# djene-mengistu/UAPS

Measured on AMD Instinct MI355X. Metric: training images/sec (labeled+unlabeled) NEU-Seg 256x256 K=3, higher is better.
Workload: dtype f32

## Files before the change

### include/uaps_hip.h

```cpp
#ifndef UAPS_HIP_H
#define UAPS_HIP_H

#include <stddef.h>
#include <stdint.h>

#ifdef __cplusplus
extern "C" {
#endif

typedef void* uaps_stream_t;

#define UAPS_MAX_HEADS 8
#define UAPS_MAX_CLASSES 8

#define UAPS_OK 0
#define UAPS_EINVAL (-1)
#define UAPS_ERANGE (-2)
#define UAPS_EWORKSPACE (-3)
#define UAPS_ENOFORM (-4)

int uaps_abi_version(void);
const char* uaps_error_string(int code);


// ... 412 lines not shown
    float focal_alpha, focal_gamma;
    int focal_mean;
    float beta;
    float tversky_alpha, tversky_beta, eps;
} uaps_binloss_params;
#define UAPS_BIN_S_TERM 0
#define UAPS_BIN_S_LOSS 7
#define UAPS_BIN_S_BAD 8
#define UAPS_BIN_S_N 9
#define UAPS_BIN_S_P 10
#define UAPS_BIN_S_G 11
#define UAPS_BIN_S_I 12
#define UAPS_BIN_S_GP 13
#define UAPS_BIN_S_GI 14
#define UAPS_BIN_S_KBCE 15
#define UAPS_BIN_S_KFOCAL 16
#define UAPS_BIN_S_NSCALARS 24
int uaps_binloss_workspace_bytes(int B, int H, int W, size_t* out_host);
int uaps_binloss_fwd(const float* z, const void* target, const uaps_binloss_params* prm, int B, int H, int W, float* scalars,
                     void* workspace, size_t workspace_bytes, uaps_stream_t stream);
int uaps_binloss_bwd(const float* z, const void* target, const uaps_binloss_params* prm, const float* scalars, const float* grad,
                     int B, int H, int W, float* dz, uaps_stream_t stream);
int uaps_sigmoid_mse_fwd(const float* a, const float* b, long n, float* out, uaps_stream_t stream);
int uaps_sigmoid_mse_bwd(const float* a, const float* b, const float* g_map, long n, float* da, uaps_stream_t stream);
int uaps_sigmoid_kl_fwd(const float* a, const float* b, long n, float* out_mean, void* workspace, size_t workspace_bytes,
                        uaps_stream_t stream);
int uaps_sigmoid_kl_bwd(const float* a, const float* b, const float* grad, long n, float* da, uaps_stream_t stream);
int uaps_bin_confusion(const float* z, const int64_t* labels, int B, int H, int W, double threshold, int64_t* counts,
                       uaps_stream_t stream);

int uaps_add_relu(const float* a, const float* b, float* out, long n, uaps_stream_t stream);
int uaps_relu_bwd(const float* dout, const float* out, float* dx, long n, uaps_stream_t stream);
int uaps_bn_act_bwd_prepare(const float* dout, const float* y, const float* gamma, const float* beta, const float* save_mean,
                            const float* save_invstd, float slope, int B, int C, int H, int W, int groups, float* coef,
                            float* dgamma, float* dbeta, float* dconv_bias, float* dy_bound, void* workspace, size_t workspace_bytes,
                            uaps_stream_t stream);
int uaps_bn_act_bwd_finalize(const void* partials, int parts_per_image, const float* maxes, const float* gamma, const float* beta,
                             const float* save_mean, const float* save_invstd, int B, int C, int H, int W, int groups, float* coef,
                             float* dgamma, float* dbeta, float* dconv_bias, float* dy_bound, uaps_stream_t stream);
int uaps_bn_act_bwd_apply(const float* dout, const float* y, const float* coef, float slope, int B, int C, int H, int W, int groups,
                          float* dy, uaps_stream_t stream);
int uaps_head_bwd_fused(const float* dlogits, const float* y, const void* xf, float slope, int groups, const float* wb,
                        const float* dy_bound, float dy_mul, const float* x_bound, float x_mul, const float* save_mean,
                        const float* save_invstd, const float* gamma, const float* beta, int want_bias, int B, int Cin, int Cout,
                        int H, int W, int ks, int cfg, float* g, void* partials, float* maxes, void* workspace,
                        size_t workspace_bytes, uaps_stream_t stream);

int uaps_mid_bwd_fused(const float* dact, const float* y2, const float* coef, float slope2, int groups2, const float* y1,
                       const void* xf, float slope, int groups, const float* wb, const float* dy_bound, float dy_mul,
                       const float* x_bound, float x_mul, const float* save_mean, const float* save_invstd, const float* gamma,
                       const float* beta, int want_bias, int B, int Cin, int Cout, int H, int W, int ks, int cfg, float* g,
                       void* partials, float* maxes, void* workspace, size_t workspace_bytes, uaps_stream_t stream);

int uaps_relu_bwd_sum(const float* const* dout_host, int k, const float* out, float* dx, long n, uaps_stream_t stream);

int uaps_cat2(const float* a, const float* b, float* out, long n, uaps_stream_t stream);

int uaps_augment_batch(const uint8_t* images_hwc, const uint8_t* masks, const int* params_i, const float* params_f,
                       const float* noise, uint64_t seed, int B, int Hs, int Ws, int Ho, int Wo, const float* mean3_host,
                       const float* std3_host, float* out, int64_t* out_mask, uaps_stream_t stream);

#define UAPS_AUG_END 0
#define UAPS_AUG_BC 1
#define UAPS_AUG_NOISE 2
#define UAPS_AUG_BLUR 3
#define UAPS_AUG_BRIGHT 4
#define UAPS_AUG_CONTRAST 5
#define UAPS_AUG_SATURATE 6
#define UAPS_AUG_HUE 7
#define UAPS_AUG_PIXDROP 8
#define UAPS_AUG_GRID 9
#define UAPS_AUG_MAX_OPS 8
typedef struct uaps_view_row {
    int32_t hflip, vflip, rot_k, grid_on;
    int32_t op[UAPS_AUG_MAX_OPS];
    float a[UAPS_AUG_MAX_OPS], b[UAPS_AUG_MAX_OPS];
} uaps_view_row;
typedef struct uaps_augment_views_call {
    uint32_t struct_size;
    int32_t V, B, Hs, Ws, Cs, Ho, Wo;
    const uint8_t* images;
    const uint8_t* masks;
    const uaps_view_row* rows_host;
    const uaps_view_row* rows;
    const float* grid_ys;
    const float* grid_xs;
    const float* noise;
    const float* drop_u;
    uint64_t seed;
    float mean[3], std[3];
    float* out;
    int64_t* out_mask;
    void* workspace;
    size_t workspace_bytes;
    uaps_stream_t stream;
} uaps_augment_views_call;
int uaps_augment_views_workspace_bytes(int V, int B, int Ho, int Wo, size_t* bytes);
int uaps_augment_views(const uaps_augment_views_call* call);

int uaps_adam_step(float* const* params_host, const float* const* grads_host, float* const* exp_avg_host,
                   float* const* exp_avg_sq_host, const long* numel_host, int n, double lr, double beta1, double beta2,
                   double eps, double weight_decay, long step, uaps_stream_t stream);

int uaps_seg_confusion(const float* logits, const int64_t* labels, int B, int C, int H, int W,
                       int64_t* counts, uaps_stream_t stream);

// ... 261 lines not shown
```

### uaps_amd/_lib.py

```python
from __future__ import annotations

import ctypes as C
import os
import subprocess
import threading

from . import config

_HERE = os.path.dirname(os.path.abspath(__file__))
LIB_PATH = config.text("UAPS_HIP_LIB") or os.path.join(_HERE, "lib", "libuaps_hip.so")
CSRC = os.path.join(_HERE, "csrc")

_lock = threading.Lock()
_tls = threading.local()
_lib = None

c_float_p = C.POINTER(C.c_float)
c_void_p = C.c_void_p

_PTR = C.c_void_p
SIGNATURES = {
    "uaps_abi_version": (C.c_int, []),
    "uaps_error_string": (C.c_char_p, [C.c_int]),
    "uaps_loss_workspace_bytes": (C.c_int, [C.c_int] * 5 + [C.POINTER(C.c_size_t)]),
# ... 47 lines not shown
    "uaps_conv_fwd_bn": (C.c_int, [_PTR, _PTR, C.c_float, C.c_int] + [_PTR] * 4 + [C.c_int] * 7 + [_PTR]),
    "uaps_conv_bwd_weight_partial_bn": (C.c_int, [_PTR, _PTR, _PTR, C.c_float, C.c_int] + [C.c_int] * 8 + [_PTR, C.c_size_t, _PTR]),
    "uaps_conv_fwd_variant": (C.c_int, [C.c_int] * 7 + [C.c_char_p, C.c_size_t]),
    "uaps_conv_wrw_variant": (C.c_int, [C.c_int] * 7 + [C.c_char_p, C.c_size_t]),
    "uaps_conv_bwd_weight": (C.c_int, [_PTR] * 4 + [C.c_int] * 7 + [_PTR, C.c_size_t, _PTR]),
    "uaps_set_step_state": (C.c_int, [_PTR]),
    "uaps_next_call_hints": (C.c_int, [_PTR]),
    "uaps_conv_ex": (C.c_int, [_PTR]),
    "uaps_conv_ex_variant": (C.c_int, [_PTR, C.c_char_p, C.c_size_t]),
    "uaps_account": (C.c_int, [C.c_int]),
    "uaps_accounted_bytes": (C.c_double, []),
    "uaps_next_launch_events": (C.c_int, [_PTR, _PTR]),
    "uaps_zero_bounds": (C.c_int, [_PTR, C.c_long, _PTR]),
    "uaps_bn_param_bounds": (C.c_int, [_PTR, _PTR, _PTR, C.c_int, _PTR, _PTR]),
    "uaps_get_step_state": (C.c_void_p, []),
    "uaps_convs_pack_floats": (C.c_int, [C.c_int] * 3 + [C.POINTER(C.c_size_t), C.POINTER(C.c_size_t)]),
    "uaps_convs_pack_weights": (C.c_int, [_PTR] + [C.c_int] * 3 + [_PTR, _PTR, _PTR]),
    "uaps_convs_out_size": (C.c_int, [C.c_int] * 5 + [C.POINTER(C.c_int), C.POINTER(C.c_int)]),
    "uaps_convs_fwd": (C.c_int, [_PTR] * 3 + [C.c_int] * 8 + [_PTR]),
    "uaps_convs_bwd_data": (C.c_int, [_PTR] * 3 + [C.c_int] * 8 + [_PTR]),
    "uaps_convs_wrw_workspace_bytes": (C.c_int, [C.c_int] * 8 + [C.POINTER(C.c_size_t)]),
    "uaps_convs_bwd_weight": (C.c_int, [_PTR] * 3 + [C.c_int] * 8 + [_PTR, C.c_size_t, _PTR]),
    "uaps_maxpool3x3s2_fwd": (C.c_int, [_PTR, _PTR, _PTR, C.c_long, C.c_int, C.c_int, _PTR]),
    "uaps_maxpool3x3s2_bwd": (C.c_int, [_PTR, _PTR, _PTR, C.c_long, C.c_int, C.c_int, _PTR]),
    "uaps_space_to_depth2": (C.c_int, [_PTR, _PTR, C.c_int, C.c_int, C.c_int, C.c_int, C.c_int, _PTR]),
    "uaps_subsample2_fwd": (C.c_int, [_PTR, _PTR, C.c_long, C.c_int, C.c_int, _PTR]),
    "uaps_subsample2_bwd": (C.c_int, [_PTR, _PTR, C.c_long, C.c_int, C.c_int, _PTR]),
    "uaps_sum_tensors": (C.c_int, [_PTR, C.c_int, _PTR, C.c_long, _PTR]),
    "uaps_pair_workspace_bytes": (C.c_int, [C.POINTER(C.c_size_t)]),
    "uaps_feat_dropout_stats": (C.c_int, [_PTR] + [C.c_int] * 4 + [_PTR, C.c_size_t, _PTR]),
    "uaps_fanout_perturbed": (C.c_int, [_PTR] * 7 + [C.c_int, C.c_int, C.c_uint64, C.c_float, C.c_float] + [C.c_int] * 4 + [_PTR]),
    "uaps_augment_batch": (C.c_int, [_PTR] * 5 + [C.c_uint64] + [C.c_int] * 5 + [C.POINTER(C.c_float), C.POINTER(C.c_float), _PTR, _PTR, _PTR]),
    "uaps_augment_views_workspace_bytes": (C.c_int, [C.c_int] * 4 + [C.POINTER(C.c_size_t)]),
    "uaps_augment_views": (C.c_int, [_PTR]),
    "uaps_softmax_klmap_bwd": (C.c_int, [_PTR] * 3 + [C.c_int] * 4 + [_PTR] * 3),
    "uaps_softmax_pair_fwd": (C.c_int, [_PTR, _PTR] + [C.c_int] * 5 + [_PTR, _PTR, _PTR, _PTR, C.c_size_t, _PTR]),
    "uaps_softmax_mse_bwd": (C.c_int, [_PTR] * 3 + [C.c_int] * 4 + [_PTR, _PTR]),
    "uaps_softmax_kl_bwd": (C.c_int, [_PTR] * 3 + [C.c_int] * 4 + [_PTR, _PTR]),
    "uaps_entropy_map": (C.c_int, [_PTR] + [C.c_int] * 4 + [_PTR, _PTR, _PTR, C.c_size_t, _PTR]),
    "uaps_fanin_perturbed": (C.c_int, [_PTR] * 4 + [C.c_int, C.c_int, C.c_uint64, C.c_float, C.c_float] + [C.c_int] * 4 + [_PTR, _PTR]),
    "uaps_maxpool2x2_fwd": (C.c_int, [_PTR] + [C.c_int] * 4 + [_PTR, _PTR, _PTR]),
    "uaps_adam_step": (C.c_int, [_PTR] * 5 + [C.c_int] + [C.c_double] * 5 + [C.c_long, _PTR]),
    "uaps_add_relu": (C.c_int, [_PTR, _PTR, _PTR, C.c_long, _PTR]),
    "uaps_relu_bwd": (C.c_int, [_PTR, _PTR, _PTR, C.c_long, _PTR]),
    "uaps_relu_bwd_sum": (C.c_int, [_PTR, C.c_int, _PTR, _PTR, C.c_long, _PTR]),
    "uaps_cat2": (C.c_int, [_PTR, _PTR, _PTR, C.c_long, _PTR]),
    "uaps_bn_act_bwd_prepare": (C.c_int, [_PTR] * 6 + [C.c_float] + [C.c_int] * 5 + [_PTR] * 6 + [C.c_size_t, _PTR]),
    "uaps_bn_act_bwd_apply": (C.c_int, [_PTR] * 3 + [C.c_float] + [C.c_int] * 5 + [_PTR, _PTR]),
    "uaps_bn_act_bwd_finalize": (C.c_int, [_PTR, C.c_int] + [_PTR] * 5 + [C.c_int] * 5 + [_PTR] * 6),
    "uaps_head_bwd_fused": (C.c_int, [_PTR] * 3 + [C.c_float, C.c_int, _PTR, _PTR, C.c_float, _PTR, C.c_float] + [_PTR] * 4 + [C.c_int] * 8 +
                            [_PTR] * 4 + [C.c_size_t, _PTR]),
    "uaps_mid_bwd_fused": (C.c_int, [_PTR] * 3 + [C.c_float, C.c_int, _PTR, _PTR, C.c_float, C.c_int, _PTR, _PTR, C.c_float, _PTR, C.c_float] +
                           [_PTR] * 4 + [C.c_int] * 8 + [_PTR] * 4 + [C.c_size_t, _PTR]),
    "uaps_seg_confusion": (C.c_int, [_PTR, _PTR] + [C.c_int] * 4 + [_PTR, _PTR]),
    "uaps_ema_update": (C.c_int, [_PTR] * 3 + [C.c_int, C.c_float, C.c_float, _PTR]),
    "uaps_teacher_noise": (C.c_int, [_PTR] + [C.c_int] * 5 + [C.c_uint64, C.c_uint64, _PTR, _PTR]),
    "uaps_teacher_noise_apply": (C.c_int, [_PTR, _PTR] + [C.c_int] * 5 + [_PTR, _PTR]),
    "uaps_mc_consistency_workspace_bytes": (C.c_int, [C.POINTER(C.c_size_t)]),
    "uaps_mc_consistency_fwd": (C.c_int, [_PTR] * 3 + [C.c_int] * 5 + [C.c_float] + [_PTR] * 4 + [C.c_size_t, _PTR]),
    "uaps_mc_consistency_bwd": (C.c_int, [_PTR] * 5 + [C.c_int] * 4 + [_PTR, _PTR]),
    "uaps_cct_dct_workspace_bytes": (C.c_int, [C.POINTER(C.c_size_t)]),
    "uaps_cct_consistency_fwd": (C.c_int, [_PTR] + [C.c_int] * 6 + [_PTR, _PTR, C.c_size_t, _PTR]),
    "uaps_cct_consistency_bwd": (C.c_int, [_PTR] + [C.c_int] * 6 + [_PTR, _PTR, _PTR]),
    "uaps_rot90_batch": (C.c_int, [_PTR, _PTR] + [C.c_int] * 5 + [_PTR, _PTR, _PTR]),
    "uaps_rot_consistency_fwd": (C.c_int, [_PTR, C.c_int, _PTR] + [C.c_int] * 6 + [_PTR, _PTR, C.c_size_t, _PTR]),
    "uaps_rot_consistency_bwd": (C.c_int, [_PTR, C.c_int, _PTR] + [C.c_int] * 6 + [_PTR, _PTR, _PTR, _PTR]),
    "uaps_cps_workspace_bytes": (C.c_int, [C.c_int] * 5 + [C.POINTER(C.c_size_t)]),
    "uaps_cps_fwd": (C.c_int, [_PTR] * 3 + [C.c_int] * 5 + [C.c_float] + [_PTR] * 4 + [C.c_size_t, _PTR]),
    "uaps_cps_bwd": (C.c_int, [_PTR] * 7 + [C.c_int] * 5 + [_PTR] * 3),
    "uaps_ucc_cutmix_batch": (C.c_int, [_PTR] * 6 + [C.c_int] * 4 + [_PTR] * 3),
    "uaps_ucc_workspace_bytes": (C.c_int, [C.c_int] * 4 + [C.POINTER(C.c_size_t)]),
    "uaps_ucc_fwd": (C.c_int, [_PTR] * 3 + [C.c_int] * 4 + [C.c_float] + [_PTR] * 6 + [C.c_size_t, _PTR]),
    "uaps_ucc_bwd": (C.c_int, [_PTR] * 6 + [C.c_int] * 4 + [_PTR] * 3),
    "uaps_segloss_workspace_bytes": (C.c_int, [C.c_int] * 4 + [C.POINTER(C.c_size_t)]),
    "uaps_segloss_fwd": (C.c_int, [_PTR] * 3 + [C.c_int] * 4 + [_PTR, _PTR, C.c_size_t, _PTR]),
    "uaps_segloss_bwd": (C.c_int, [_PTR] * 5 + [C.c_int] * 4 + [_PTR, _PTR]),
    "uaps_binloss_workspace_bytes": (C.c_int, [C.c_int] * 3 + [C.POINTER(C.c_size_t)]),
    "uaps_binloss_fwd": (C.c_int, [_PTR] * 3 + [C.c_int] * 3 + [_PTR, _PTR, C.c_size_t, _PTR]),
    "uaps_binloss_bwd": (C.c_int, [_PTR] * 5 + [C.c_int] * 3 + [_PTR, _PTR]),
    "uaps_sigmoid_mse_fwd": (C.c_int, [_PTR, _PTR, C.c_long, _PTR, _PTR]),
    "uaps_sigmoid_mse_bwd": (C.c_int, [_PTR, _PTR, _PTR, C.c_long, _PTR, _PTR]),
    "uaps_sigmoid_kl_fwd": (C.c_int, [_PTR, _PTR, C.c_long, _PTR, _PTR, C.c_size_t, _PTR]),
    "uaps_sigmoid_kl_bwd": (C.c_int, [_PTR, _PTR, _PTR, C.c_long, _PTR, _PTR]),
    "uaps_bin_confusion": (C.c_int, [_PTR, _PTR] + [C.c_int] * 3 + [C.c_double, _PTR, _PTR]),
    "uaps_tta_views": (C.c_int, [_PTR]),
    "uaps_tta_fold": (C.c_int, [_PTR]),
    "uaps_instances_workspace_bytes": (C.c_int, [C.c_int] * 3 + [C.POINTER(C.c_size_t)]),
    "uaps_label_instances": (C.c_int, [_PTR]),
    "uaps_rle_count": (C.c_int, [_PTR]),
    "uaps_rle_encode": (C.c_int, [_PTR]),
    "uaps_rle_decode": (C.c_int, [_PTR]),
    "uaps_tile_origins": (C.c_int, [C.c_int] * 3 + [C.POINTER(C.c_int), C.POINTER(C.c_int), C.c_int]),
    "uaps_tile_cut": (C.c_int, [_PTR]),
    "uaps_tile_fold": (C.c_int, [_PTR]),
    "uaps_edt_workspace_bytes": (C.c_int, [C.c_int] * 3 + [C.POINTER(C.c_size_t)]),
    "uaps_edt_sq": (C.c_int, [_PTR]),
    "uaps_surface_workspace_bytes": (C.c_int, [C.c_int] * 4 + [C.POINTER(C.c_size_t)]),
    "uaps_surface_distances": (C.c_int, [_PTR]),
    "uaps_match_workspace_bytes": (C.c_int, [C.c_int] * 3 + [C.POINTER(C.c_size_t)]),
    "uaps_match_instances": (C.c_int, [_PTR]),
    "uaps_curves_workspace_bytes": (C.c_int, [C.c_int] * 3 + [C.POINTER(C.c_size_t)]),
    "uaps_score_curves": (C.c_int, [_PTR]),
    "uaps_plane_curves": (C.c_int, [_PTR]),
}


# ... 368 lines not shown
```

### uaps_amd/config.py

```python
from __future__ import annotations

import os
from typing import Dict

_seen: Dict[str, tuple] = {}

DOC = {
    "UAPS_HIP_LIB": "path of another build of libuaps_hip.so with the same ABI (same-box A/B of two kernel builds)",
    "UAPS_CONV_MODE": "arithmetic of the convolutions: 2 / h16 (default), 1 / split (exact three-piece bf16), 0 / exact (fp32 MFMA)",
    "UAPS_DEFER_WRW_REDUCE": "weight-gradient reductions batched behind the backward (conv.deferred_reduces)",
    "UAPS_EARLY_WRW_REDUCE": "... and the decoders' share of them on a side stream beside the encoder's backward",
    "UAPS_EARLY_ADAM": "the decoders' Adam step behind their early reductions (world size 1)",
    "UAPS_FUSED_UP2": "bilinear x2 formed in the staging of up4's first convolution instead of materialised",
    "UAPS_FUSED_BN_SUMS": "BatchNorm-backward sums in the epilogue of the 16 -> 16 input-gradient row kernel (measured a wash: off)",
    "UAPS_FUSED_HEAD_BWD": "out_conv's input gradient, weight gradient and the BatchNorm-backward sums behind it as one row pass (csrc/head_bwd_row.hip)",
    "UAPS_FUSED_MID_BWD": "the 16 -> 16 convolution of a 256-wide ConvBlock: weight gradient, input gradient and the BatchNorm-backward sums behind it as one row pass (csrc/mid_bwd_row.hip)",
    "UAPS_LAZY_BN_BWD": "BatchNorm backward in two halves on the 256-wide decoder layers (lazybn)",
    "UAPS_PAIR_CFG": "cfg bits of the pair-loss kernels (diagnosis)",
    "UAPS_FUSED_FANOUT": "all perturbed copies of a feature map written by one pass over it",
    "UAPS_EPILOGUE_STATS": "BatchNorm statistics in the producing convolution's epilogue",
    "UAPS_VIRTUAL_CAT": "two-source convolutions instead of a materialised torch.cat in the UpBlocks",
    "UAPS_FUSED_FAN": "perturbation backward fused into the gradient fan-in kernel",
    "UAPS_DECODER_CHAINS": "decoders are dealt round-robin onto this many streams (diagnosis)",
    "UAPS_FAN_BESIDE": "perturbed feature copies written on a side stream beside the encoder's next levels",
    "UAPS_PACK_BESIDE": "the decoders' weights packed on a side stream beside the encoder's forward",
    "UAPS_FUSED_POOL": "2x2 max-pool fused into the fan-out / fan-in kernels",
    "UAPS_FUSED_BN_CONV": "BatchNorm + LeakyReLU applied in the consuming convolution's staging",
    "UAPS_DECODER_STREAMS": "one HIP stream per auxiliary decoder (bench.py switches it on for the headline)",
    "UAPS_STAT_SHIFT": "BatchNorm partial sums formed about running_mean - conv bias",
    "UAPS_INPUT_IN_GRAPH": "the captured step reads the batch from its own static input buffers (filled by the concatenation kernel)",
}


def _raw(name: str):
    return os.environ.get(name)


def flag(name: str, default: bool) -> bool:
    v = _raw(name)
    val = default if v is None or v == "" else (v != "0")
    _seen[name] = (default, val)
    return val


def integer(name: str, default: int) -> int:
    v = _raw(name)
    val = default if v is None or v == "" else int(v)
    _seen[name] = (default, val)
    return val


def text(name: str, default=None):
    v = _raw(name)
    val = default if v is None or v == "" else v
    _seen[name] = (default, val)
    return val


def non_default() -> Dict[str, object]:
    out = {k: v for k, (d, v) in sorted(_seen.items()) if v != d}
    for k in sorted(os.environ):
        if k.startswith("UAPS_") and k not in _seen:
            out[k] = os.environ[k]
    return out
```

### uaps_amd/conv.py

```python
from __future__ import annotations

import collections
import contextlib
import ctypes as C
import os
import weakref
from typing import Dict, Optional, Tuple

import torch
from torch.optim.optimizer import register_optimizer_step_post_hook

from . import _graddest, lazybn, _lib, bounds, config, stepctx

_ws = _lib.Workspace(min_bytes=1 << 22)
_packed: Dict[int, tuple] = {}
_generation = 0
_shared_cell = [0]


def optimizer_stepped(optimizer, *_args, **_kwargs) -> None:
    cell = getattr(optimizer, "_uaps_cell", None)
    if cell is None:
        cell = optimizer._uaps_cell = [0]
    cell[0] += 1
# ... 558 lines not shown
        st = _lib.current_stream(dev)
        _lib.check(L.uaps_zero_bounds(maxes.data_ptr(), maxes.numel(), st), "uaps_zero_bounds")
        with (_lib.LaunchTimer() if on else contextlib.nullcontext()) as timer:
            rc = L.uaps_head_bwd_fused(dz.data_ptr(), y.data_ptr(), xf.data_ptr(), float(slope), int(groups), wb.data_ptr(),
                                       dzb[0].data_ptr() if dzb is not None else None, float(dzb[1]) if dzb is not None else 1.0,
                                       xb[0].data_ptr() if xb is not None else None, float(xb[1]) if xb is not None else 1.0,
                                       mean.data_ptr(), invstd.data_ptr(), gamma.data_ptr(), beta.data_ptr(), int(want_bias), B, Cin, Cout,
                                       H, W, 3, cfg, g.data_ptr(), partials.data_ptr(), maxes.data_ptr(), ws.data_ptr(), ws.numel(), st)
        if on and rc == 0:
            KERNEL_EVENTS.setdefault(HEAD_BWD_KERNEL, []).append((timer.start, timer.stop, 2 * 2.0 * B * H * W * Cin * Cout * 9))
    if rc == ENOFORM:
        return None
    _lib.check(rc, "uaps_head_bwd_fused")
    return g, partials, maxes


_FUSED_MID = config.flag("UAPS_FUSED_MID_BWD", True)
MID_BWD_KERNEL = "mid_bwd_row_kernel"


def mid_bwd_eligible(dz: torch.Tensor, y: torch.Tensor, ks: int) -> bool:
    return (_FUSED_MID and ks == 3 and y.shape[1] == 16 and dz.shape[1] == 16 and y.shape[3] == 256 and y.shape[2] % 16 == 0
            and get_mode() == "h16")


def mid_bwd_fused(dz: torch.Tensor, lz, y: torch.Tensor, xf: torch.Tensor, xb, wb: torch.Tensor, mean, invstd, gamma, beta,
                  slope: float, groups: int, want_bias: bool, cfg: int, ws: torch.Tensor):
    B, Cout, H, W = dz.shape
    Cin = y.shape[1]
    dev = y.device
    g = torch.empty_like(y)
    partials = torch.empty((Cin, B, max(H // 16, 1), 2), dtype=torch.float32, device=dev)
    maxes = torch.empty(2 * bounds.FLOATS, dtype=torch.float32, device=dev)
    dzb = lz.bound if lz is not None else None
    L = _lib.lib()
    on = KERNEL_EVENTS is not None and (EVENT_FILTER is None or MID_BWD_KERNEL in EVENT_FILTER)
    with _lib.device_guard(dev):
        st = _lib.current_stream(dev)
        _lib.check(L.uaps_zero_bounds(maxes.data_ptr(), maxes.numel(), st), "uaps_zero_bounds")
        with (_lib.LaunchTimer() if on else contextlib.nullcontext()) as timer:
            rc = L.uaps_mid_bwd_fused(dz.data_ptr(), lz.y.data_ptr() if lz is not None else None, lz.coef.data_ptr() if lz is not None else None,
                                      float(lz.slope) if lz is not None else 0.0, int(lz.groups) if lz is not None else 1,
                                      y.data_ptr(), xf.data_ptr(), float(slope), int(groups), wb.data_ptr(),
                                      dzb[0].data_ptr() if dzb is not None else None, float(dzb[1]) if dzb is not None else 1.0,
                                      xb[0].data_ptr() if xb is not None else None, float(xb[1]) if xb is not None else 1.0,
                                      mean.data_ptr(), invstd.data_ptr(), gamma.data_ptr(), beta.data_ptr(), int(want_bias), B, Cin, Cout,
                                      H, W, 3, cfg, g.data_ptr(), partials.data_ptr(), maxes.data_ptr(), ws.data_ptr(), ws.numel(), st)
        if on and rc == 0:
            KERNEL_EVENTS.setdefault(MID_BWD_KERNEL, []).append((timer.start, timer.stop, 2 * 2.0 * B * H * W * Cin * Cout * 9))
    if rc == ENOFORM:
        return None
    _lib.check(rc, "uaps_mid_bwd_fused")
    return g, partials, maxes


def conv_bwd_weight_raw(dy: torch.Tensor, x: torch.Tensor, ks: int, want_bias: bool, cfg: int = 0, wkey=None, bkey=None,
                        dyb=None, xb=None, lz=None, prefs=None, step=None):
    B, Cout, H, W = dy.shape
    Cin = x.shape[1]
    dev = dy.device
    L = _lib.lib()
    n = C.c_size_t()
    cfg = plan_cfg(ks, cfg, True, dy, x)
    _lib.check(L.uaps_conv_wrw_workspace_bytes(B, Cin, Cout, H, W, ks, cfg, C.byref(n)), "uaps_conv_wrw_workspace_bytes")
    ws = _wrw_workspace(dev, n.value, prefs, step)
    dw = _graddest.take(wkey, (Cout, Cin, ks, ks), dev)
    db = _graddest.take(bkey, (Cout,), dev) if want_bias else None
    dy_true = None
    with _lib.device_guard(dev):
        st = _lib.current_stream(dev)
        rc = lazybn.ENOFORM
        if lz is not None and xb is not None:
            dy_true = torch.empty_like(dy)
            hh = _lib.mk_hints((lz.bound, xb), dyt=(lz.y, lz.coef, dy_true, lz.slope, lz.groups))
            with _timed(WRW, B, Cin, Cout, H, W, ks, cfg, hh, y_grad=dy, x=x):
                rc = L.uaps_conv_bwd_weight_partial_h(hh, dy.data_ptr(), x.data_ptr(), int(want_bias), B, Cin, Cout, H, W, ks, cfg,
                                                      ws.data_ptr(), ws.numel(), st)
            if rc != lazybn.ENOFORM:
                bounds.put(dy_true, *lz.bound)
        if lz is not None and rc == lazybn.ENOFORM:
            dy_true = dy = lazybn.materialize(dy, lz)
            dyb = bounds.get(dy)
        if lz is None or rc == lazybn.ENOFORM:
            hh = _lib.mk_hints((dyb, xb)) if (dyb is not None and xb is not None) else None
            with _timed(WRW, B, Cin, Cout, H, W, ks, cfg, hh, y_grad=dy, x=x):
                rc = L.uaps_conv_bwd_weight_partial_h(hh, dy.data_ptr(), x.data_ptr(), int(want_bias), B, Cin, Cout, H, W, ks, cfg,
                                                      ws.data_ptr(), ws.numel(), st)
        _lib.check(rc, "uaps_conv_bwd_weight_partial")
        _wrw_reduce(ws, dw, db, B, Cin, Cout, H, W, ks, cfg, st, prefs, step)
    if lz is not None:
        return dw, db, dy_true
    return dw, db


def _dil_cfg(dilation: int) -> int:
    if dilation not in (1, 2, 4):
        raise ValueError("conv2d: dilation 1, 2 or 4")
    return 0 if dilation == 1 else dilation << 24


class _Conv2d(torch.autograd.Function):
    @staticmethod
    def forward(ctx, x, weight, bias, want_stats=False, dilation=1, stat_shift=None):
        _lib.require_device(x, "conv2d")
        ctx.set_materialize_grads(False)
        if x.dtype != torch.float32 or weight.dtype != torch.float32:
# ... 108 lines not shown
        C1, C2, Cout, ks, has_bias, cfg = ctx.meta
        up2 = ctx.up2
        ucfg = cfg | (X2_UP2 if up2 else 0)
        x2w = x2
        lz = lazybn.take(dy)
        dyb = bounds.get(dy)
        b1, b2 = ctx.xb
        dy = dy.contiguous()
        B, _, H, W = dy.shape
        dev = dy.device
        L = _lib.lib()
        st = _lib.current_stream(dev)
        dx1 = dx2 = dw = db = None
        want_db = has_bias and ctx.needs_input_grad[3]
        want_w = ctx.needs_input_grad[2] or want_db
        if up2 and want_w and (b1 is None or b2 is None or (lz is None and dyb is None)):
            x2w = torch.empty((B, C2, H, W), dtype=torch.float32, device=dev)
            with _lib.device_guard(dev):
                _lib.check(L.uaps_up_cat_fwd(x2.data_ptr(), x2.data_ptr(), x2w.data_ptr(), B, 0, C2, H // 2, W // 2, st), "uaps_up_cat_fwd")
            ucfg = cfg

        def weight_gradient(dy, dyb, lz):
            n = C.c_size_t()
            _lib.check(L.uaps_conv_wrw_workspace_bytes(B, C1 + C2, Cout, H, W, ks, cfg, C.byref(n)), "uaps_conv_wrw_workspace_bytes")
            ws = _wrw_workspace(dev, n.value, ctx.prefs, ctx.step)
            dw = _graddest.take(ctx.keys[0], (Cout, C1 + C2, ks, ks), dev)
            db = _graddest.take(ctx.keys[1], (Cout,), dev) if want_db else None
            out = torch.empty_like(dy) if lz is not None else None
            hh = None
            if lz is not None:
                hh = _lib.mk_hints((dyb, b1, b2), dyt=(lz.y, lz.coef, out, lz.slope, lz.groups))
            elif dyb is not None and b1 is not None and b2 is not None:
                hh = _lib.mk_hints((dyb, b1, b2))
            with _timed(WRW, B, C1 + C2, Cout, H, W, ks, ucfg, hh, y_grad=dy, x=x1, C1=C1, x2=x2w):
                rc = L.uaps_conv_bwd_weight_partial_cat_h(hh, dy.data_ptr(), x1.data_ptr(), C1, x2w.data_ptr(), C2, int(want_db), B, Cout,
                                                          H, W, ks, ucfg, ws.data_ptr(), ws.numel(), st)
            if lz is not None and rc == lazybn.ENOFORM:
                return None, None, None
            _lib.check(rc, "uaps_conv_bwd_weight_partial_cat")
            _wrw_reduce(ws, dw, db, B, C1 + C2, Cout, H, W, ks, cfg, st, ctx.prefs, ctx.step)
            return dw, db, (bounds.put(out, *lz.bound) if lz is not None else dy)

        with _lib.device_guard(dev):
            done_w = False
            if lz is not None:
                if want_w and b1 is not None and b2 is not None:
                    dw, db, out = weight_gradient(dy, lz.bound, lz)
                    done_w = out is not None
                if done_w:
                    dy = out
                else:
                    dy = lazybn.materialize(dy, lz)
                dyb = bounds.get(dy)
            if ctx.needs_input_grad[0] or ctx.needs_input_grad[1]:
                dx1 = torch.empty_like(x1)
                dx2 = torch.empty((B, C2, H, W), dtype=torch.float32, device=dev) if up2 else torch.empty_like(x2)
                hh = _lib.mk_hints((dyb,)) if dyb is not None else None
                with _timed(BWD_DATA, B, C1 + C2, Cout, H, W, ks, cfg, hh, x=dy, y=dx1, C1=C1, y2=dx2):
                    rc = L.uaps_conv_bwd_data_cat_h(hh, dy.data_ptr(), wb.data_ptr(), dx1.data_ptr(), C1, dx2.data_ptr(), C2, B, Cout, H, W,
                                                    ks, cfg, st)
                _lib.check(rc, "uaps_conv_bwd_data_cat")
            if want_w and not done_w:
                dw, db, _ = weight_gradient(dy, dyb, None)
            if up2 and dx2 is not None:
                dlow = torch.empty_like(x2)
                rc = L.uaps_up_cat_bwd(dx2.data_ptr(), None, dlow.data_ptr(), B, 0, C2, H // 2, W // 2, st)
                _lib.check(rc, "uaps_up_cat_bwd")
                dx2 = dlow
        return dx1, dx2, dw, db, None, None, None


def conv2d_cat(x1: torch.Tensor, x2: torch.Tensor, weight: torch.Tensor, bias: Optional[torch.Tensor] = None,
               with_stats: bool = False, stat_shift=None, up2: bool = False):
    res = _Conv2dCat.apply(x1, x2, weight, bias, with_stats, stat_shift, up2)
    return _mark(res, stat_shift is not None, weight) if with_stats else res



_spacked: Dict[int, tuple] = {}


def _pack_strided(weight: torch.Tensor):
    key = id(weight)
    ent = _spacked.get(key)
    if ent is not None and ent[0]() is weight and ent[1] == weight._version and ent[2] == stamp(weight) and ent[3].device == weight.device:
        return ent[3], ent[4]
    Cout, Cin, ks, ks2 = weight.shape
    nf, nb = C.c_size_t(), C.c_size_t()
    L = _lib.lib()
    _lib.check(L.uaps_convs_pack_floats(Cout, Cin, ks, C.byref(nf), C.byref(nb)), "uaps_convs_pack_floats")
    dev = weight.device
    wf = torch.empty(nf.value, dtype=torch.float32, device=dev)
    wb = torch.empty(nb.value, dtype=torch.float32, device=dev)
    w = weight.detach().contiguous()
    with _lib.device_guard(dev):
        rc = L.uaps_convs_pack_weights(w.data_ptr(), Cout, Cin, ks, wf.data_ptr(), wb.data_ptr(), _lib.current_stream(dev))
    _lib.check(rc, "uaps_convs_pack_weights")
    _spacked[key] = (weakref.ref(weight), weight._version, stamp(weight), wf, wb)
    return wf, wb


class _ConvStrided(torch.autograd.Function):

    @staticmethod
    def forward(ctx, x, weight, stride, padding):
        _lib.require_device(x, "conv2d_strided")
        if x.dtype != torch.float32 or weight.dtype != torch.float32:
            raise TypeError("conv2d_strided: fp32 only")
        x = x.contiguous()
        B, Cin, H, W = x.shape
        Cout, Cin2, ks, ks2 = weight.shape
        if Cin2 != Cin or ks != ks2:
            raise ValueError(f"conv2d_strided: input has {Cin} channels, weight is {tuple(weight.shape)}")
        wf, wb = _pack_strided(weight)
        L = _lib.lib()
        oh, ow = C.c_int(), C.c_int()
        _lib.check(L.uaps_convs_out_size(H, W, ks, stride, padding, C.byref(oh), C.byref(ow)), "uaps_convs_out_size")
# ... 156 lines not shown
```

Baseline: 2762.

## Fold up-sampled half of up4 input gradient into row kernel

Adds a fused HIP row kernel for the first convolution of up4 that computes the input gradient for both the skip half and the up-sampled half. It folds the up-sampled half's gradient back to low resolution with bilinear weights inside the kernel, rather than writing a full-resolution dx2 and running a separate up_cat_bwd pass. This is meant to remove a full-resolution intermediate write and read plus one kernel launch. In exchange it adds a specialised kernel that only handles 16-channel, 256-wide, h16-mode shapes, and it changes the rounding order of the fold reduction.

New measurement: 2793, median of 6. 1.01x the previous value.

```diff
diff --git a/include/uaps_hip.h b/include/uaps_hip.h
--- a/include/uaps_hip.h
+++ b/include/uaps_hip.h
@@ -488,6 +488,12 @@
                        const float* beta, int want_bias, int B, int Cin, int Cout, int H, int W, int ks, int cfg, float* g,
                        void* partials, float* maxes, void* workspace, size_t workspace_bytes, uaps_stream_t stream);
 
+int uaps_up_bwd_fused(const float* dy, const float* wb, const float* dy_bound, float dy_mul, float* dskip, int C1, float* dlow, int C2,
+                      int B, int Cout, int H, int W, int ks, int cfg, uaps_stream_t stream);
+int uaps_up_fold_support(int n_in, int* min_offset, int* max_offset);
+int uaps_up_bwd_fused_form(int H, int W);
+int uaps_up_bwd_fused_grid(int B, int H);
+
 int uaps_relu_bwd_sum(const float* const* dout_host, int k, const float* out, float* dx, long n, uaps_stream_t stream);
 
 int uaps_cat2(const float* a, const float* b, float* out, long n, uaps_stream_t stream);
diff --git a/uaps_amd/_lib.py b/uaps_amd/_lib.py
--- a/uaps_amd/_lib.py
+++ b/uaps_amd/_lib.py
@@ -123,6 +123,10 @@
                             [_PTR] * 4 + [C.c_size_t, _PTR]),
     "uaps_mid_bwd_fused": (C.c_int, [_PTR] * 3 + [C.c_float, C.c_int, _PTR, _PTR, C.c_float, C.c_int, _PTR, _PTR, C.c_float, _PTR, C.c_float] +
                            [_PTR] * 4 + [C.c_int] * 8 + [_PTR] * 4 + [C.c_size_t, _PTR]),
+    "uaps_up_bwd_fused": (C.c_int, [_PTR, _PTR, _PTR, C.c_float, _PTR, C.c_int, _PTR] + [C.c_int] * 7 + [_PTR]),
+    "uaps_up_fold_support": (C.c_int, [C.c_int, C.POINTER(C.c_int), C.POINTER(C.c_int)]),
+    "uaps_up_bwd_fused_form": (C.c_int, [C.c_int, C.c_int]),
+    "uaps_up_bwd_fused_grid": (C.c_int, [C.c_int, C.c_int]),
     "uaps_seg_confusion": (C.c_int, [_PTR, _PTR] + [C.c_int] * 4 + [_PTR, _PTR]),
     "uaps_ema_update": (C.c_int, [_PTR] * 3 + [C.c_int, C.c_float, C.c_float, _PTR]),
     "uaps_teacher_noise": (C.c_int, [_PTR] + [C.c_int] * 5 + [C.c_uint64, C.c_uint64, _PTR, _PTR]),
diff --git a/uaps_amd/config.py b/uaps_amd/config.py
--- a/uaps_amd/config.py
+++ b/uaps_amd/config.py
@@ -15,6 +15,7 @@
     "UAPS_FUSED_BN_SUMS": "BatchNorm-backward sums in the epilogue of the 16 -> 16 input-gradient row kernel (measured a wash: off)",
     "UAPS_FUSED_HEAD_BWD": "out_conv's input gradient, weight gradient and the BatchNorm-backward sums behind it as one row pass (csrc/head_bwd_row.hip)",
     "UAPS_FUSED_MID_BWD": "the 16 -> 16 convolution of a 256-wide ConvBlock: weight gradient, input gradient and the BatchNorm-backward sums behind it as one row pass (csrc/mid_bwd_row.hip)",
+    "UAPS_FUSED_UP_FOLD": "the input gradient of up4's first convolution folds its up-sampled half to the low resolution inside the row kernel (csrc/up_bwd_row.hip)",
     "UAPS_LAZY_BN_BWD": "BatchNorm backward in two halves on the 256-wide decoder layers (lazybn)",
     "UAPS_PAIR_CFG": "cfg bits of the pair-loss kernels (diagnosis)",
     "UAPS_FUSED_FANOUT": "all perturbed copies of a feature map written by one pass over it",
diff --git a/uaps_amd/conv.py b/uaps_amd/conv.py
--- a/uaps_amd/conv.py
+++ b/uaps_amd/conv.py
@@ -634,6 +634,37 @@
         return None
     _lib.check(rc, "uaps_mid_bwd_fused")
     return g, partials, maxes
+
+
+_FUSED_UP_FOLD = config.flag("UAPS_FUSED_UP_FOLD", True)
+UP_BWD_KERNEL = "up_bwd_row_kernel"
+
+
+def up_bwd_eligible(dy: torch.Tensor, C1: int, C2: int, ks: int) -> bool:
+    return (_FUSED_UP_FOLD and ks == 3 and dy.shape[1] == 16 and C1 == 16 and C2 == 16 and dy.shape[3] == 256 and dy.shape[2] % 16 == 0
+            and get_mode() == "h16")
+
+
+def up_bwd_fused(dy: torch.Tensor, dyb, wb: torch.Tensor, C1: int, C2: int, cfg: int):
+    B, Cout, H, W = dy.shape
+    dev = dy.device
+    if dyb is None:
+        return None
+    dskip = torch.empty((B, C1, H, W), dtype=torch.float32, device=dev)
+    dlow = torch.empty((B, C2, H // 2, W // 2), dtype=torch.float32, device=dev)
+    L = _lib.lib()
+    on = KERNEL_EVENTS is not None and (EVENT_FILTER is None or UP_BWD_KERNEL in EVENT_FILTER)
+    with _lib.device_guard(dev):
+        st = _lib.current_stream(dev)
+        with (_lib.LaunchTimer() if on else contextlib.nullcontext()) as timer:
+            rc = L.uaps_up_bwd_fused(dy.data_ptr(), wb.data_ptr(), dyb[0].data_ptr(), float(dyb[1]), dskip.data_ptr(), C1, dlow.data_ptr(), C2,
+                                     B, Cout, H, W, 3, cfg, st)
+        if on and rc == 0:
+            KERNEL_EVENTS.setdefault(UP_BWD_KERNEL, []).append((timer.start, timer.stop, 2.0 * B * H * W * (C1 + C2) * Cout * 9))
+    if rc == ENOFORM:
+        return None
+    _lib.check(rc, "uaps_up_bwd_fused")
+    return dskip, dlow
 
 
 def conv_bwd_weight_raw(dy: torch.Tensor, x: torch.Tensor, ks: int, want_bias: bool, cfg: int = 0, wkey=None, bkey=None,
@@ -848,7 +879,12 @@
                 else:
                     dy = lazybn.materialize(dy, lz)
                 dyb = bounds.get(dy)
-            if ctx.needs_input_grad[0] or ctx.needs_input_grad[1]:
+            folded = None
+            if (ctx.needs_input_grad[0] or ctx.needs_input_grad[1]) and up2 and up_bwd_eligible(dy, C1, C2, ks):
+                folded = up_bwd_fused(dy, dyb, wb, C1, C2, cfg)
+            if folded is not None:
+                dx1, dx2 = folded
+            elif ctx.needs_input_grad[0] or ctx.needs_input_grad[1]:
                 dx1 = torch.empty_like(x1)
                 dx2 = torch.empty((B, C2, H, W), dtype=torch.float32, device=dev) if up2 else torch.empty_like(x2)
                 hh = _lib.mk_hints((dyb,)) if dyb is not None else None
@@ -858,7 +894,7 @@
                 _lib.check(rc, "uaps_conv_bwd_data_cat")
             if want_w and not done_w:
                 dw, db, _ = weight_gradient(dy, dyb, None)
-            if up2 and dx2 is not None:
+            if up2 and dx2 is not None and folded is None:
                 dlow = torch.empty_like(x2)
                 rc = L.uaps_up_cat_bwd(dx2.data_ptr(), None, dlow.data_ptr(), B, 0, C2, H // 2, W // 2, st)
                 _lib.check(rc, "uaps_up_cat_bwd")
diff --git a/uaps_amd/csrc/up_bwd_row.hip b/uaps_amd/csrc/up_bwd_row.hip
--- /dev/null
+++ b/uaps_amd/csrc/up_bwd_row.hip
@@ -0,0 +1,300 @@
+#include "../../include/uaps_hip.h"
+#include "conv_kernels.hpp"
+#include "conv_split.hpp"
+#include "hints.hpp"
+#include "up2_staging.hpp"
+
+extern "C" int uaps_conv_get_mode(void);
+extern "C" unsigned uaps_conv_get_tuning(void);
+
+namespace uaps {
+
+typedef unsigned u32x2 __attribute__((ext_vector_type(2)));
+
+struct UpBwdArgs {
+    const float* dy;
+    const float* wp;
+    const float* wscale;
+    int CGP;
+    float* dskip;
+    float* dlow;
+    const float* dy_bound; float dy_mul;
+    float rh, rw;
+    unsigned* err;
+    int B, H, nsplit;
+};
+
+__device__ __forceinline__ float up_fold_weight(float r, int o, int n_out, int n_in, int i) {
+    if (o < 0 || o >= n_out) return 0.f;
+    const float sx = mul_rn(r, (float)o);
+    const int i0 = (int)sx, i1 = i0 + (i0 < n_in - 1 ? 1 : 0);
+    const float l1 = sx - (float)i0, l0 = 1.f - l1;
+    return (i0 == i ? l0 : 0.f) + (i1 == i ? l1 : 0.f);
+}
+
+__global__ __launch_bounds__(512, 2) void up_bwd_row_kernel(UpBwdArgs a) {
+    constexpr int WIDTH = 256, NSLOT = 3, ROWS = 16, NTHR = 512, NCH = 4;
+    constexpr int IW = WIDTH + 8, CGU = NSLOT * IW, PIECE = 2 * CGU, XS = 3;
+    constexpr int NQ = 9 * 2, NSTEP = (NQ + 3) / 4, MW = 4, CoutP = 32;
+    constexpr int GS = WIDTH + 4;
+
+    __shared__ __attribute__((aligned(16))) u32x4 sIn[2 * PIECE];
+    __shared__ __attribute__((aligned(16))) float sG[2][16 * GS];
+
+    const f32x2 sc = h16_scale(__builtin_fmaxf(bound_of(a.dy_bound, a.dy_mul), 0.f));
+    const float in_scale = sc.x, out_scale_a = sc.y, out_scale_w = a.wscale[1];
+
+    const int tid = threadIdx.x, lane = tid & 63, wave = tid >> 6;
+    const int j = lane & 15, kq = lane >> 4;
+    const int wave_u = __builtin_amdgcn_readfirstlane(wave);
+    const bool is_up = wave_u >= 4;
+    const int half = wave_u >> 2, wq = wave_u & 3;
+    const int W = WIDTH, HW = a.H * W, h = a.H / 2, w = WIDTH / 2;
+    const uint32_t HW4 = (uint32_t)HW * 4u, hw4 = (uint32_t)(h * w) * 4u;
+
+    const int split = xcd_swizzle(blockIdx.x, gridDim.x);
+    if (split >= a.nsplit) return;
+    const int rpi = a.H / ROWS, nruns = a.B * rpi;
+    const int run_begin = (int)((long)nruns * split / a.nsplit), run_end = (int)((long)nruns * (split + 1) / a.nsplit);
+
+    for (int e = tid; e < 2 * 2 * NSLOT * 8; e += NTHR) sIn[(e / 8) * IW + (e % 8 < 4 ? e % 8 : IW - 8 + e % 8)] = u32x4{0u, 0u, 0u, 0u};
+
+    u32x4 bfr[NSTEP][2];
+    int kxo[NSTEP], kyv[NSTEP];
+    {
+        const __amdgpu_buffer_rsrc_t rs_w = make_rsrc(a.wp, (uint32_t)(2 * 9) * a.CGP * CoutP * 16u);
+#pragma unroll
+        for (int s = 0; s < NSTEP; ++s) {
+            const int q = 4 * s + kq, tap = q / 2, cgq = q % 2;
+#pragma unroll
+            for (int p = 0; p < 2; ++p) {
+                const uint32_t off = q < NQ ? (uint32_t)(((p * 9 + tap) * a.CGP + cgq) * CoutP + half * 16 + j) * 16u : kOob;
+                bfr[s][p] = __builtin_amdgcn_raw_buffer_load_b128(rs_w, (int)off, 0, 0);
+            }
+            const int qq = q < NQ ? q : 0;
+            kxo[s] = (qq % 2) * CGU + (qq / 2) % 3; kyv[s] = (qq / 2) / 3;
+        }
+    }
+    int abase[MW];
+#pragma unroll
+    for (int m = 0; m < MW; ++m) abase[m] = (wq * MW + m) * 16 + j + XS;
+
+    const int dc0 = wq * NCH, cg = wq >> 1, ch = wq & 1;
+    f32x4 rd[NCH];
+    auto ld4 = [](__amdgpu_buffer_rsrc_t rs, uint32_t off) { return __builtin_bit_cast(f32x4, __builtin_amdgcn_raw_buffer_load_b128(rs, (int)off, 0, 0)); };
+    auto load_d = [&](int b, int gy, f32x4 (&dd)[NCH]) {
+        const bool ok = (unsigned)gy < (unsigned)a.H;
+        const __amdgpu_buffer_rsrc_t rs = make_rsrc(a.dy + (size_t)b * 16 * HW, 16u * HW4);
+        const uint32_t off = (uint32_t)(dc0 * HW + gy * W + lane * 4) * 4u;
+#pragma unroll
+        for (int i = 0; i < NCH; ++i) dd[i] = ld4(rs, ok ? off + (uint32_t)i * HW4 : kOob);
+    };
+    auto store_d = [&](f32x4 (&dd)[NCH], int slot) {
+#pragma unroll
+        for (int i = 0; i < NCH; ++i) asm volatile("" : "+v"(dd[i]));
+        const int base = (cg * NSLOT + slot) * IW + 4 + lane * 4;
+#pragma unroll
+        for (int k = 0; k < 4; ++k) {
+            unsigned q00, q01, q10, q11;
+            conv_split2h(dd[0][k] * in_scale, dd[1][k] * in_scale, q00, q01);
+            conv_split2h(dd[2][k] * in_scale, dd[3][k] * in_scale, q10, q11);
+            *reinterpret_cast<uint2*>(reinterpret_cast<unsigned*>(&sIn[base + k]) + ch * 2) = make_uint2(q00, q10);
+            *reinterpret_cast<uint2*>(reinterpret_cast<unsigned*>(&sIn[PIECE + base + k]) + ch * 2) = make_uint2(q01, q11);
+        }
+    };
+
+    float wxa[4], wxb[4];
+#pragma unroll
+    for (int k = 0; k < 4; ++k) {
+        wxa[k] = up_fold_weight(a.rw, 4 * lane - 1 + k, W, w, 2 * lane);
+        wxb[k] = up_fold_weight(a.rw, 4 * lane + 1 + k, W, w, 2 * lane + 1);
+    }
+    float accp[NCH][2], accq[NCH][2];
+#pragma unroll
+    for (int i = 0; i < NCH; ++i) { accp[i][0] = accp[i][1] = 0.f; accq[i][0] = accq[i][1] = 0.f; }
+
+    for (int run = run_begin; run < run_end; ++run) {
+        const int b = run / rpi, r0 = (run % rpi) * ROWS;
+        if (!is_up) {
+            f32x4 da[NCH], db[NCH];
+            load_d(b, r0 - 2, da);
+            load_d(b, r0 - 1, db);
+            load_d(b, r0, rd);
+            __builtin_amdgcn_sched_barrier(0);
+            store_d(da, 0);
+            store_d(db, 1);
+            store_d(rd, 2);
+        }
+        __syncthreads();
+        int s0 = 0;
+        const __amdgpu_buffer_rsrc_t rs_g = make_rsrc(a.dskip + (size_t)b * 16 * HW, 16u * HW4);
+        const __amdgpu_buffer_rsrc_t rs_l = make_rsrc(a.dlow + (size_t)b * 16 * h * w, 16u * hw4);
+#pragma unroll 1
+        for (int t = r0 - 1; t <= r0 + ROWS; ++t) {
+            const bool more = t < r0 + ROWS;
+            if (!is_up && more) load_d(b, t + 2, rd);
+            const int s1 = s0 + 1 >= NSLOT ? s0 + 1 - NSLOT : s0 + 1, s2 = s1 + 1 >= NSLOT ? s1 + 1 - NSLOT : s1 + 1;
+            const bool own = t >= r0 && t < r0 + ROWS;
+            const bool work = is_up ? (unsigned)t < (unsigned)a.H : own;
+
+            f32x4 gacc[MW];
+#pragma unroll
+            for (int m = 0; m < MW; ++m) gacc[m] = f32x4{0.f, 0.f, 0.f, 0.f};
+            if (work) {
+                int aoff[NSTEP];
+#pragma unroll
+                for (int s = 0; s < NSTEP; ++s) aoff[s] = kxo[s] + (kyv[s] == 0 ? s0 : (kyv[s] == 1 ? s1 : s2)) * IW;
+                constexpr int NUN = NSTEP * MW;
+                u32x4 af[2][2];
+                auto read_a = [&](int u, u32x4 (&dst)[2]) {
+                    const int s = u / MW, m = u % MW;
+#pragma unroll
+                    for (int p = 0; p < 2; ++p) dst[p] = sIn[p * PIECE + abase[m] + aoff[s]];
+                };
+                read_a(0, af[0]);
+#pragma unroll
+                for (int u = 0; u < NUN; ++u) {
+                    const int s = u / MW, m = u % MW;
+                    if (u + 1 < NUN) read_a(u + 1, af[(u + 1) & 1]);
+                    const auto Hf = [](const u32x4& v) { return __builtin_bit_cast(f16x8, v); };
+                    f32x4 c = gacc[m];
+                    c = __builtin_amdgcn_mfma_f32_16x16x32_f16(Hf(af[u & 1][1]), Hf(bfr[s][0]), c, 0, 0, 0);
+                    c = __builtin_amdgcn_mfma_f32_16x16x32_f16(Hf(af[u & 1][0]), Hf(bfr[s][1]), c, 0, 0, 0);
+                    c = __builtin_amdgcn_mfma_f32_16x16x32_f16(Hf(af[u & 1][0]), Hf(bfr[s][0]), c, 0, 0, 0);
+                    gacc[m] = c;
+                    if (u + 1 < NUN) __builtin_amdgcn_sched_group_barrier(0x100, 2, 0);
+                    __builtin_amdgcn_sched_group_barrier(0x008, 3, 0);
+                }
+            }
+            float chk = 0.f;
+#pragma unroll
+            for (int m = 0; m < MW; ++m) {
+                f32x4 v = gacc[m];
+                v *= out_scale_a; v *= out_scale_w;
+                v += 0.f;
+                note_nonfinite(chk, v);
+                *reinterpret_cast<f32x4*>(&sG[half][j * GS + (wq * MW + m) * 16 + kq * 4]) = v;
+            }
+            report_nonfinite(a.err, chk, UAPS_ERR_CONV_NONFINITE);
+            __syncthreads();
+
+            if (!is_up) {
+                if (own) {
+#pragma unroll
+                    for (int i = 0; i < NCH; ++i) {
+                        const f32x4 gv = *reinterpret_cast<const f32x4*>(&sG[0][(dc0 + i) * GS + lane * 4]);
+                        __builtin_amdgcn_raw_buffer_store_b128(__builtin_bit_cast(u32x4, gv), rs_g, (int)((uint32_t)((dc0 + i) * HW + t * W + lane * 4) * 4u), 0, 0);
+                    }
+                }
+                if (more) store_d(rd, s0);
+            } else {
+                const bool odd = (t & 1) != 0;
+                const int ip = odd ? (t - 1) / 2 : t / 2 - 1, iq = ip + 1;
+                const float wyp = up_fold_weight(a.rh, t, a.H, h, ip), wyq = up_fold_weight(a.rh, t, a.H, h, iq);
+                const bool out = !odd && t > r0;
+#pragma unroll
+                for (int i = 0; i < NCH; ++i) {
+                    const f32x4 gv = *reinterpret_cast<const f32x4*>(&sG[1][(dc0 + i) * GS + lane * 4]);
+                    const float prev = up2_lane_prev(gv[3]), next = up2_lane_next(gv[0]);
+                    float ta = mul_rn(wxa[0], prev);
+                    ta = add_rn(ta, mul_rn(wxa[1], gv[0])); ta = add_rn(ta, mul_rn(wxa[2], gv[1])); ta = add_rn(ta, mul_rn(wxa[3], gv[2]));
+                    float tb = mul_rn(wxb[0], gv[1]);
+                    tb = add_rn(tb, mul_rn(wxb[1], gv[2])); tb = add_rn(tb, mul_rn(wxb[2], gv[3])); tb = add_rn(tb, mul_rn(wxb[3], next));
+                    accp[i][0] = add_rn(accp[i][0], mul_rn(wyp, ta)); accp[i][1] = add_rn(accp[i][1], mul_rn(wyp, tb));
+                    if (odd) { accq[i][0] = mul_rn(wyq, ta); accq[i][1] = mul_rn(wyq, tb); }
+                    else { accq[i][0] = add_rn(accq[i][0], mul_rn(wyq, ta)); accq[i][1] = add_rn(accq[i][1], mul_rn(wyq, tb)); }
+                    if (!odd) {
+                        const f32x2 lo = f32x2{accp[i][0], accp[i][1]};
+                        __builtin_amdgcn_raw_buffer_store_b64(__builtin_bit_cast(u32x2, lo), rs_l,
+                                                              (int)(out ? (uint32_t)((dc0 + i) * h * w + ip * w + lane * 2) * 4u : kOob), 0, 0);
+                        accp[i][0] = accq[i][0]; accp[i][1] = accq[i][1];
+                    }
+                }
+            }
+            s0 = s1;
+            __syncthreads();
+        }
+    }
+}
+
+}
+
+namespace {
+void fold_support(int n_in, int* lo, int* hi) {
+    const int n_out = 2 * n_in;
+    const float r = n_out > 1 ? (float)(n_in - 1) / (float)(n_out - 1) : 0.f;
+    int mn = n_out, mx = -n_out;
+    for (int o = 0; o < n_out; ++o) {
+        volatile float sx = r * (float)o;
+        const float s = sx;
+        const int i0 = (int)s, i1 = i0 + (i0 < n_in - 1 ? 1 : 0);
+        volatile float l1v = s - (float)i0;
+        const float l1 = l1v;
+        volatile float l0v = 1.f - l1;
+        const float l0 = l0v;
+        const int is[2] = {i0, i1};
+        const float ws[2] = {i0 == i1 ? l0 + l1 : l0, i0 == i1 ? 0.f : l1};
+        for (int k = 0; k < 2; ++k) {
+            if (ws[k] == 0.f) continue;
+            const int d = o - 2 * is[k];
+            if (d < mn) mn = d;
+            if (d > mx) mx = d;
+        }
+    }
+    *lo = mn; *hi = mx;
+}
+}
+
+extern "C" int uaps_up_fold_support(int n_in, int* min_offset, int* max_offset) {
+    if (n_in <= 0 || n_in > (1 << 20) || !min_offset || !max_offset) return UAPS_EINVAL;
+    fold_support(n_in, min_offset, max_offset);
+    return UAPS_OK;
+}
+
+extern "C" int uaps_up_bwd_fused_form(int H, int W) {
+    if (H <= 0 || W <= 0) return UAPS_EINVAL;
+    if (W != 256 || H % 16 || H > 65536) return UAPS_ENOFORM;
+    int lo = 0, hi = 0;
+    fold_support(H / 2, &lo, &hi);
+    if (lo < -1 || hi > 2) return UAPS_ENOFORM;
+    fold_support(W / 2, &lo, &hi);
+    if (lo < -1 || hi > 2) return UAPS_ENOFORM;
+    return UAPS_OK;
+}
+
+extern "C" int uaps_up_bwd_fused_grid(int B, int H) {
+    if (B <= 0 || H <= 0 || H % 16) return UAPS_EINVAL;
+    const long nruns = (long)B * (H / 16);
+    return (int)(nruns < 256 ? nruns : 256);
+}
+
+extern "C" int uaps_up_bwd_fused(const float* dy, const float* wb, const float* dy_bound, float dy_mul, float* dskip, int C1, float* dlow,
+                                 int C2, int B, int Cout, int H, int W, int ks, int cfg, uaps_stream_t stream) {
+    if (!dy || !wb || !dskip || !dlow) return UAPS_EINVAL;
+    if (B <= 0 || C1 <= 0 || C2 <= 0 || Cout <= 0 || H <= 0 || W <= 0) return UAPS_EINVAL;
+    if (ks != 3 || Cout != 16 || C1 != 16 || C2 != 16 || W != 256 || H % 16 || H > 65536 || (cfg & ~UAPS_CONV_BOUNDED)) return UAPS_ENOFORM;
+    if ((long)B * (H / 16) > 0x7fffffffL) return UAPS_ENOFORM;
+    if (uaps_conv_get_mode() != 2 || !dy_bound) return UAPS_ENOFORM;
+    if (uaps_conv_get_tuning() & (UAPS_TUNE_NO_SPLIT_FWD | UAPS_TUNE_NO_HP16 | UAPS_TUNE_NO_ROW16)) return UAPS_ENOFORM;
+    if (((uintptr_t)dy | (uintptr_t)wb | (uintptr_t)dskip | (uintptr_t)dlow) % 16) return UAPS_ENOFORM;
+    const int rc = uaps_up_bwd_fused_form(H, W);
+    if (rc) return rc;
+    uaps::account_bytes(4.0 * B * H * W * (1.0 * Cout + 1.0 * C1 + 0.25 * C2));
+    uaps::UpBwdArgs a{};
+    a.dy = dy;
+    const int CGP = uaps::split_cgroups(Cout), CoP = 32;
+    const float* split_w = wb + (size_t)9 * ((Cout + 7) / 8 * 8) * CoP;
+    const size_t piece = (size_t)9 * CGP * CoP * 4;
+    a.wscale = split_w + 3 * piece + 16;
+    a.wp = split_w + 3 * piece + uaps::kH16Header;
+    a.CGP = CGP;
+    a.dskip = dskip; a.dlow = dlow;
+    a.dy_bound = dy_bound; a.dy_mul = dy_mul;
+    a.rh = (float)(H / 2 - 1) / (float)(H - 1); a.rw = (float)(W / 2 - 1) / (float)(W - 1);
+    a.err = uaps::error_word();
+    a.B = B; a.H = H;
+    a.nsplit = uaps_up_bwd_fused_grid(B, H);
+    const unsigned grid = (unsigned)((a.nsplit + 7) / 8 * 8);
+    UAPS_LAUNCH_MAIN(uaps::up_bwd_row_kernel, dim3(grid), dim3(512), 0, (hipStream_t)stream, a);
+    return (int)hipGetLastError();
+}
```
